# jianhao2016/AllSet

Measured on AMD Instinct MI355X. Metric: edges*d aggregated / sec (V->E->V layer fwd+bwd), higher is better.
Workload: dtype f32

## Files before the change

### allset_amd/csrc/fused_fwd2.hip

```cpp
#include <stdlib.h>

#include "common.h"
#include "mfma.h"

namespace allset {

constexpr int kF2Block = 768;
constexpr int kF2Rows = 32;
constexpr int kF2VWaves = 8;
constexpr int kF2Sets = 4;

#ifdef ALLSET_ABL5_NOBAR
#define ALLSET_TICK() ALLSET_TICK_NO_BARRIER()
#else
#define ALLSET_TICK() ALLSET_TICK_BARRIER()
#endif

template <bool HAS_LN, bool DROP_IN, bool DROP_OUT, bool D8, bool F16, int XM = 0, bool AUX = false>
__global__ __launch_bounds__(kF2Block) void fused_linear_fwd_roles_kernel(
    const float* __restrict__ x, int64_t ldx, const float* __restrict__ gamma, const float* __restrict__ beta, float eps,
    int relu_in, float p_in, uint64_t seed_in, const float* __restrict__ W, const float* __restrict__ bias, int relu_out,
    float p_out, uint64_t seed_out, float* __restrict__ y, int64_t ldy, float* __restrict__ stats, int64_t n,
    const uint64_t* __restrict__ seed_base, uint32_t* __restrict__ mask_out, int64_t xcb, int64_t ycb, float ln_inv,
    const float* __restrict__ colb = nullptr, float* __restrict__ uo = nullptr, int64_t lduo = 0,
// ... 275 lines not shown
        if constexpr (XM == 3 || XM == 4) vv[hb] = v;
#ifdef ALLSET_ABL5_NOSTORE
        if (live && v.x == 123.456f)
#else
        if (live && XM != 2 && XM != 3 && XM != 4)
#endif
          *reinterpret_cast<float4*>(yb + hb * dhy + yo) = v;
        if (mask_out != nullptr) {
          const uint64_t b0 = __ballot(v.x > 0.f), b1 = __ballot(v.y > 0.f), b2 = __ballot(v.z > 0.f), b3 = __ballot(v.w > 0.f);
          const int sh = 8 * (lane0 & 7);
          const uint32_t word = static_cast<uint32_t>((b0 >> sh) & 0xffu) | (static_cast<uint32_t>((b1 >> sh) & 0xffu) << 8) |
                                (static_cast<uint32_t>((b2 >> sh) & 0xffu) << 16) | (static_cast<uint32_t>((b3 >> sh) & 0xffu) << 24);
          if (lane0 < 8 && 16 * (wave >> 2) < nrows)
            mask_out[((stage * (R / 16) + (wave >> 2)) * (ND / 64) + hb) * 32 + (wave & 3) * 8 + lane0] = word;
        }
      }
      if constexpr (XM == 3 || XM == 4) {
        uint32_t u[2][4], own[2] = {0u, 0u}, oth[2] = {0u, 0u};
        int pos[2], kocc;
        const uint32_t sh = 4u * (c & 7);
        const bool hi = c >= 8;
#pragma unroll
        for (int hb = 0; hb < 2; ++hb) {
          u[hb][0] = __float_as_uint(vv[hb].x); u[hb][1] = __float_as_uint(vv[hb].y);
          u[hb][2] = __float_as_uint(vv[hb].z); u[hb][3] = __float_as_uint(vv[hb].w);
        }
        if constexpr (XM == 4) {
          int n2[2];
#pragma unroll
          for (int hb = 0; hb < 2; ++hb)
            n2[hb] = ((u[hb][0] != 0u ? 1 : 0) + (u[hb][1] != 0u ? 1 : 0)) + ((u[hb][2] != 0u ? 1 : 0) + (u[hb][3] != 0u ? 1 : 0));
          const int pk = n2[0] | (n2[1] << 8);
          int inc = pk, tot = pk;
          inc += __builtin_amdgcn_update_dpp(0, inc, 0x111, 0xf, 0xf, true);
          inc += __builtin_amdgcn_update_dpp(0, inc, 0x112, 0xf, 0xf, true);
          inc += __builtin_amdgcn_update_dpp(0, inc, 0x114, 0xf, 0xf, true);
          inc += __builtin_amdgcn_update_dpp(0, inc, 0x118, 0xf, 0xf, true);
          tot += __builtin_amdgcn_update_dpp(0, tot, 0xB1, 0xf, 0xf, false);
          tot += __builtin_amdgcn_update_dpp(0, tot, 0x4E, 0xf, 0xf, false);
          tot += __builtin_amdgcn_update_dpp(0, tot, 0x141, 0xf, 0xf, false);
          tot += __builtin_amdgcn_update_dpp(0, tot, 0x140, 0xf, 0xf, false);
          const int exc = inc - pk, cnt0 = tot & 0xff;
          kocc = cnt0 + (tot >> 8);
          pos[0] = 4 + (exc & 0xff);
          pos[1] = 4 + cnt0 + (exc >> 8);
        } else {
#pragma unroll
          for (int hb = 0; hb < 2; ++hb) {
            const uint32_t nib = (u[hb][0] != 0u ? 1u : 0u) | (u[hb][1] != 0u ? 2u : 0u) | (u[hb][2] != 0u ? 4u : 0u) | (u[hb][3] != 0u ? 8u : 0u);
            float mw = __uint_as_float(nib << sh);
            mw = __uint_as_float(__float_as_uint(mw) | __float_as_uint(dpp_row<0xB1>(mw)));
            mw = __uint_as_float(__float_as_uint(mw) | __float_as_uint(dpp_row<0x4E>(mw)));
            mw = __uint_as_float(__float_as_uint(mw) | __float_as_uint(dpp_row<0x141>(mw)));
            own[hb] = __float_as_uint(mw);
            oth[hb] = __float_as_uint(dpp_row<0x140>(mw));
          }
          const uint32_t below = (1u << sh) - 1u;
          const int cnt0 = __popc(own[0]) + __popc(oth[0]);
          kocc = cnt0 + __popc(own[1]) + __popc(oth[1]);
          pos[0] = 4 + (hi ? __popc(oth[0]) : 0) + __popc(own[0] & below);
          pos[1] = 4 + cnt0 + (hi ? __popc(oth[1]) : 0) + __popc(own[1] & below);
        }
        uint32_t* im = reinterpret_cast<uint32_t*>(sY + (k & 1) * (R * SPY) + lr * SPY);
        __builtin_amdgcn_fence(__ATOMIC_SEQ_CST, "wavefront");
        __builtin_amdgcn_wave_barrier();
        if constexpr (XM == 4) {
          static_assert(kCellCap == 48 && kCellCap + 3 < 64 && 64 + kCellCap + 3 < SPY, "three slots per cell; the staged columns sit 64 dwords above the values");
          const uint32_t dcol = 128u + c;
#pragma unroll
          for (int s = 0; s < 3; ++s) { im[16 * s + c] = 0u; im[64 + 16 * s + c] = dcol; }
#pragma unroll
          for (int hb = 0; hb < 2; ++hb) {
            int j = min(pos[hb] - 4, kCellCap);
#pragma unroll
            for (int i = 0; i < 4; ++i) {
              const bool occ = u[hb][i] != 0u;
              const int at = occ ? j : kCellCap;
              im[at] = u[hb][i];
              im[64 + at] = static_cast<uint32_t>(64 * hb + 4 * c + i);
              j += occ ? 1 : 0;
            }
          }
        } else {
        *reinterpret_cast<uint4*>(im + 4 * c) = make_uint4(0u, 0u, 0u, 0u);
        *reinterpret_cast<uint4*>(im + (hi ? SPY - 4 : 0)) = make_uint4(own[0], oth[0], own[1], oth[1]);
#pragma unroll
        for (int hb = 0; hb < 2; ++hb)
#pragma unroll
          for (int i = 0; i < 4; ++i) {
            const bool occ = u[hb][i] != 0u;
            im[occ ? pos[hb] : SPY - 1] = u[hb][i];
            pos[hb] += occ ? 1 : 0;
          }
        }
        __builtin_amdgcn_fence(__ATOMIC_SEQ_CST, "wavefront");
        __builtin_amdgcn_wave_barrier();
        uint4 o;
        if constexpr (XM == 4)
          o = make_uint4(im[c], im[16 + c], im[32 + c], (im[64 + c] | (im[80 + c] << 8)) | ((im[96 + c] | (static_cast<uint32_t>(kocc) << 8)) << 16));
        else
          o = *reinterpret_cast<const uint4*>(im + 4 * c);
        if (live) *reinterpret_cast<uint4*>(reinterpret_cast<uint32_t*>(uo) + (stage * R + lr) * kPackPitchDw + 4 * c) = o;
        if (live && kocc > (XM == 4 ? kCellCap : kPackCap)) {
          *reinterpret_cast<float4*>(yb + yo) = vv[0];
          *reinterpret_cast<float4*>(yb + 256 + yo) = vv[1];
        }
      }
      if constexpr (XM == 2) {
        __builtin_amdgcn_sched_barrier(0);
        request_res(k + 1);
        __builtin_amdgcn_sched_barrier(0);
      }
    };

    static_assert(kF2Sets == 4, "the trip below is written for four register sets");
#pragma unroll
    for (int q = 0; q < kF2Sets; ++q) request_x(q, xrS[q]);
    request_res(0);
    S0(0, xrS[0]);
    ALLSET_TICK();
    S0(1, xrS[1]);
    ALLSET_TICK();
#define ALLSET_F2_FULL_TICK(tt, set) do { ALLSET_MARK(3); S0((tt) + 1, xrS[set]); ALLSET_MARK(0); E((tt) - 1, eC); ALLSET_MARK(1); ALLSET_TICK(); ALLSET_MARK(2); } while (0)
    int64_t t = 1;
    for (; t + 3 < T; t += 4) {
      ALLSET_F2_FULL_TICK(t, 2);
      ALLSET_F2_FULL_TICK(t + 1, 3);
      ALLSET_F2_FULL_TICK(t + 2, 0);
      ALLSET_F2_FULL_TICK(t + 3, 1);
    }
    if (t < T) ALLSET_F2_FULL_TICK(t, 2);
    if (t + 1 < T) ALLSET_F2_FULL_TICK(t + 1, 3);
    if (t + 2 < T) ALLSET_F2_FULL_TICK(t + 2, 0);
#undef ALLSET_F2_FULL_TICK
    E(T - 1, eB);
  } else {
    const int m = wave - kF2VWaves;
    Frag wq[2][4][F16 ? 2 : 3];
    float inv_s = 1.f;
    if constexpr (F16) {
      const int nn = lane0 & 15, kg = lane0 >> 4;
      float4 wa[2][4], wb[2][4];
      float amax = 0.f;
#pragma unroll
      for (int ct = 0; ct < 2; ++ct)
#pragma unroll
        for (int tt = 0; tt < 4; ++tt) {
          const float4* wr = reinterpret_cast<const float4*>(W + (32 * m + 16 * ct + nn) * KD + 32 * kg + 8 * tt);
          wa[ct][tt] = wr[0]; wb[ct][tt] = wr[1];
          amax = fmaxf(fmaxf(fmaxf(fabsf(wa[ct][tt].x), fabsf(wa[ct][tt].y)), fmaxf(fabsf(wa[ct][tt].z), fabsf(wa[ct][tt].w))), amax);
          amax = fmaxf(fmaxf(fmaxf(fabsf(wb[ct][tt].x), fabsf(wb[ct][tt].y)), fmaxf(fabsf(wb[ct][tt].z), fabsf(wb[ct][tt].w))), amax);
        }
#pragma unroll
      for (int off = 1; off < 64; off <<= 1) amax = fmaxf(amax, __shfl_xor(amax, off));
      const int ew = __builtin_amdgcn_readfirstlane(min(max(static_cast<int>(__float_as_uint(amax) >> 23), 20), 254));
      const float sw = __uint_as_float(static_cast<uint32_t>(254 + 13 - ew) << 23);
      const int X = ew - 140 - Su, X1 = X >> 1, X2 = X - X1;
      inv_s = __uint_as_float(static_cast<uint32_t>(127 + X1) << 23) * __uint_as_float(static_cast<uint32_t>(127 + X2) << 23);
#pragma unroll
      for (int ct = 0; ct < 2; ++ct)
#pragma unroll
        for (int tt = 0; tt < 4; ++tt) {
          const float4 a = wa[ct][tt], b = wb[ct][tt];
          uint32_t ph[4], pl[4];
          split2_f16(a.x * sw, a.y * sw, ph[0], pl[0]);
          split2_f16(a.z * sw, a.w * sw, ph[1], pl[1]);
          split2_f16(b.x * sw, b.y * sw, ph[2], pl[2]);
          split2_f16(b.z * sw, b.w * sw, ph[3], pl[3]);
          wq[ct][tt][0].u = make_uint4(ph[0], ph[1], ph[2], ph[3]);
          wq[ct][tt][1].u = make_uint4(pl[0], pl[1], pl[2], pl[3]);
        }
    } else {
      const int nn = lane0 & 15, kg = lane0 >> 4;
#pragma unroll
      for (int ct = 0; ct < 2; ++ct)
#pragma unroll
// ... 299 lines not shown
```

### allset_amd/csrc/segreduce.hip

```cpp
#include "common.h"
#include "flat_rows.h"
#include "mfma.h"

namespace allset {

enum { kModeSum = 0, kModeExt = 1 };
constexpr int kUnroll = 8;
#ifndef ALLSET_SEG_UNROLL_ONE_SLOT
#define ALLSET_SEG_UNROLL_ONE_SLOT 8
#endif
#ifndef ALLSET_SEG_MAX_LPR
#define ALLSET_SEG_MAX_LPR 64
#endif
constexpr int kBwdUnroll = 4;

template <typename T, int VEC, int LPR, int MODE, bool WEIGHTED>
__global__ __launch_bounds__(kBlock) void segreduce_kernel(
    const int32_t* __restrict__ rowptr, const int32_t* __restrict__ col, const float* __restrict__ w,
    const T* __restrict__ x, int64_t ldx, T* __restrict__ out, int64_t ldo,
    int32_t* __restrict__ argext, int n_t, int d, int mean, float sign, const int32_t* __restrict__ row_order) {
  constexpr int NS = kWave / LPR;
  constexpr int U = NS == 1 ? ALLSET_SEG_UNROLL_ONE_SLOT : kUnroll;
  const unsigned blk = xcd_contiguous_block(blockIdx.x, gridDim.x);
  const int slot_row = static_cast<int>(blk) * kWavesPerBlock + (threadIdx.x >> 6);
// ... 275 lines not shown
        const int jj = j + u * NS + slot;
        const int src = __shfl(my_col, jj & (kWave - 1));
        if (jj < n && active) raw[u] = load_raw<float, VEC>(x + static_cast<int64_t>(src) * ldx + c0);
        else raw[u] = zero_raw<float, VEC>();
      }
      float res = 0.f;
#pragma unroll
      for (int u = 0; u < kUnroll; ++u) {
        const FVec<VEC> v = unpack<float, VEC>(raw[u]);
        float part = 0.f;
#pragma unroll
        for (int k = 0; k < VEC; ++k) {
          if constexpr (MODE == kModeExt) part = (ap[k] == base + j + u * NS + slot) ? fmaf(v.v[k], g.v[k], part) : part;
          else part = fmaf(v.v[k], g.v[k], part);
        }
        part = slot_sum<LPR>(part);
        res = (li == u) ? part : res;
      }
      const int jo = j + li * NS + slot;
      if (li < kUnroll && jo < n) gw[base + jo] = res * scale;
    }
  }
}

constexpr int kPackRowsPerWave = 4;
constexpr int kExpand = 2;

__device__ __forceinline__ void lds_wave_handoff() {
  __builtin_amdgcn_fence(__ATOMIC_SEQ_CST, "wavefront");
  __builtin_amdgcn_wave_barrier();
}

__device__ __forceinline__ uint32_t all_ones_if_bit(uint32_t m, int b) {
  return static_cast<uint32_t>(__builtin_amdgcn_sbfe(static_cast<int>(m), static_cast<unsigned>(b), 1u));
}

__device__ __forceinline__ int mask_count(const uint4& m) { return __popc(m.x) + __popc(m.y) + __popc(m.z) + __popc(m.w); }

template <bool CELLS>
__global__ __launch_bounds__(kBlock) void pack_kernel(const float* __restrict__ x, int64_t ldx, uint32_t* __restrict__ packed, int64_t n) {
  __shared__ __attribute__((aligned(16))) uint32_t image[kWavesPerBlock][kPackRowsPerWave][kPackPitchDw];
  const int wave = threadIdx.x >> 6, lane = lane_id();
  const int slot = lane >> 5, li = lane & 31;
  const int64_t row0 = (static_cast<int64_t>(blockIdx.x) * kWavesPerBlock + wave) * kPackRowsPerWave;
  if (row0 >= n) return;
  uint4 raw[kPackRowsPerWave / 2];
#pragma unroll
  for (int p = 0; p < kPackRowsPerWave / 2; ++p) {
    const int64_t r = row0 + 2 * p + slot;
    raw[p] = r < n ? *reinterpret_cast<const uint4*>(x + r * ldx + 4 * li) : make_uint4(0u, 0u, 0u, 0u);
  }
#pragma unroll
  for (int p = 0; p < kPackRowsPerWave / 2; ++p) {
    uint32_t* dst = image[wave][2 * p + slot];
    const uint32_t v[4] = {raw[p].x, raw[p].y, raw[p].z, raw[p].w};
    const unsigned nib = (v[0] != 0u ? 1u : 0u) | (v[1] != 0u ? 2u : 0u) | (v[2] != 0u ? 4u : 0u) | (v[3] != 0u ? 8u : 0u);
    const int g = li >> 3, sh = 4 * (li & 7);
    unsigned mw = nib << sh;
    mw |= __shfl_xor(mw, 1);
    mw |= __shfl_xor(mw, 2);
    mw |= __shfl_xor(mw, 4);
    uint4 m;
    m.x = __shfl(mw, slot * 32);
    m.y = __shfl(mw, slot * 32 + 8);
    m.z = __shfl(mw, slot * 32 + 16);
    m.w = __shfl(mw, slot * 32 + 24);
    int j = (g > 0 ? __popc(m.x) : 0) + (g > 1 ? __popc(m.y) : 0) + (g > 2 ? __popc(m.z) : 0) + __popc(mw & ((1u << sh) - 1u));
    if constexpr (CELLS) {
      uint8_t* dstb = reinterpret_cast<uint8_t*>(dst);
      const uint32_t k = static_cast<uint32_t>(mask_count(m));
      if (li < kCellsPerRow) *reinterpret_cast<uint4*>(dst + 4 * li) = make_uint4(0u, 0u, 0u, (128u + li) * 0x010101u | (k << 24));
      lds_wave_handoff();
#pragma unroll
      for (int i = 0; i < 4; ++i) {
        if ((nib >> i) & 1u) {
          if (j < kCellCap) {
            dst[4 * (j & 15) + (j >> 4)] = v[i];
            dstb[16 * (j & 15) + 12 + (j >> 4)] = static_cast<uint8_t>(4 * li + i);
          }
          ++j;
        }
      }
    } else {
      int pos = 4 + j;
#pragma unroll
      for (int i = 0; i < 4; ++i) {
        if ((nib >> i) & 1u) {
          if (pos < kPackPitchDw) dst[pos] = v[i];
          ++pos;
        }
      }
      if (li == 0) *reinterpret_cast<uint4*>(dst) = m;
    }
  }
  lds_wave_handoff();
  const int rr = lane >> 4, q = 4 * (lane & 15);
  const uint32_t* src = image[wave][rr];
  uint4 o = *reinterpret_cast<const uint4*>(src + q);
  if constexpr (!CELLS) {
    const int k = mask_count(*reinterpret_cast<const uint4*>(src));
    if (q + 0 >= 4 + k) o.x = 0u;
    if (q + 1 >= 4 + k) o.y = 0u;
    if (q + 2 >= 4 + k) o.z = 0u;
    if (q + 3 >= 4 + k) o.w = 0u;
  }
  if (row0 + rr < n) *reinterpret_cast<uint4*>(packed + (row0 + rr) * kPackPitchDw + q) = o;
}

constexpr int kImagePad = 128;
__global__ __launch_bounds__(kBlock) __attribute__((amdgpu_waves_per_eu(8, 8))) void segreduce_packed_kernel(
    const int32_t* __restrict__ rowptr, const int32_t* __restrict__ col, const uint32_t* __restrict__ packed,
    const float* __restrict__ x, int64_t ldx, float* __restrict__ out, int64_t ldo, int n_t, int mean,
    const int32_t* __restrict__ row_order) {
  constexpr int VEC = 4, LPR = 32, NS = 2, U = kUnroll;
  __shared__ __attribute__((aligned(16))) uint32_t image[kWavesPerBlock * U * NS * kPackPitchDw + kImagePad];
  const unsigned blk = xcd_contiguous_block(blockIdx.x, gridDim.x);
  const int slot_row = static_cast<int>(blk) * kWavesPerBlock + (threadIdx.x >> 6);
  if (slot_row >= n_t) return;
  const int row = row_order ? row_order[slot_row] : slot_row;
  const int wave = threadIdx.x >> 6, lane = lane_id();
  const int slot = lane / LPR, li = lane % LPR;
  const int start = rowptr[row], end = rowptr[row + 1];
  const uint32_t below = (1u << li) - 1u;
  uint32_t* const mine = image + (wave * U * NS + slot) * kPackPitchDw;
  float acc[VEC];
#pragma unroll
  for (int g = 0; g < VEC; ++g) acc[g] = 0.f;

  for (int base = start; base < end; base += kWave) {
    const int n = min(kWave, end - base);
    int my_col = 0;
    if (lane < n) my_col = col[base + lane];
    for (int j = 0; j < n; j += NS * U) {
      uint2 raw[U];
#pragma unroll
      for (int u = 0; u < U; ++u) {
        const int jj = j + u * NS + slot;
        const int src = __shfl(my_col, jj & (kWave - 1));
        if (jj < n) raw[u] = *reinterpret_cast<const uint2*>(packed + static_cast<int64_t>(src) * kPackPitchDw + 2 * li);
        else raw[u] = make_uint2(0u, 0u);
      }
#pragma unroll
      for (int u = 0; u < U; ++u) *reinterpret_cast<uint2*>(mine + u * NS * kPackPitchDw + 2 * li) = raw[u];
      lds_wave_handoff();
#pragma unroll
      for (int u0 = 0; u0 < U; u0 += kExpand) {
        if (j + u0 * NS >= n) break;
        uint4 m[kExpand];
#pragma unroll
        for (int e = 0; e < kExpand; ++e) m[e] = *reinterpret_cast<const uint4*>(mine + (u0 + e) * NS * kPackPitchDw);
        uint32_t v[kExpand][VEC];
        bool over[kExpand];
        bool any_over = false;
#pragma unroll
        for (int e = 0; e < kExpand; ++e) {
          const uint32_t* r = mine + (u0 + e) * NS * kPackPitchDw;
          const int c1 = 4 + __popc(m[e].x), c2 = c1 + __popc(m[e].y), c3 = c2 + __popc(m[e].z);
          over[e] = c3 + __popc(m[e].w) > 4 + kPackCap;
          any_over |= over[e];
          v[e][0] = r[4 + __popc(m[e].x & below)] & all_ones_if_bit(m[e].x, li);
          v[e][1] = r[c1 + __popc(m[e].y & below)] & all_ones_if_bit(m[e].y, li);
          v[e][2] = r[c2 + __popc(m[e].z & below)] & all_ones_if_bit(m[e].z, li);
          v[e][3] = r[c3 + __popc(m[e].w & below)] & all_ones_if_bit(m[e].w, li);
        }
        if (__any(any_over)) {
#pragma unroll
          for (int e = 0; e < kExpand; ++e) {
            const int src = __shfl(my_col, (j + (u0 + e) * NS + slot) & (kWave - 1));
            if (over[e]) {
              const uint32_t* xr = reinterpret_cast<const uint32_t*>(x + static_cast<int64_t>(src) * ldx) + li;
#pragma unroll
              for (int g = 0; g < VEC; ++g) v[e][g] = xr[32 * g];
            }
          }
        }
#pragma unroll
        for (int e = 0; e < kExpand; ++e)
#pragma unroll
          for (int g = 0; g < VEC; ++g) acc[g] = fmaf(1.f, __uint_as_float(v[e][g]), acc[g]);
      }
      lds_wave_handoff();
    }
  }

#pragma unroll
  for (int off = LPR; off < kWave; off <<= 1)
#pragma unroll
    for (int g = 0; g < VEC; ++g) acc[g] += __shfl_xor(acc[g], off);

  if (slot == 0) {
    const float scale = mean ? 1.f / static_cast<float>(max(end - start, 1)) : 1.f;
    float* o = out + static_cast<int64_t>(row) * ldo + li;
#pragma unroll
    for (int g = 0; g < VEC; ++g) o[32 * g] = acc[g] * scale;
  }
}

#ifndef ALLSET_CELL_WAVES
#define ALLSET_CELL_WAVES 8
#endif
constexpr int kCellImageDw = 128 + kCellsPerRow;

__device__ __forceinline__ float add_value_first(uint32_t v, float acc) {
  float r;
  asm("v_add_f32 %0, %1, %2" : "=v"(r) : "v"(v), "v"(acc));
  return r;
}

template <int Q, int H>
__global__ __launch_bounds__(kBlock) __attribute__((amdgpu_waves_per_eu(ALLSET_CELL_WAVES, ALLSET_CELL_WAVES))) void segreduce_cells_kernel(
    const int32_t* __restrict__ rowptr, const int32_t* __restrict__ col, const uint4* __restrict__ cells,
    const float* __restrict__ x, int64_t ldx, float* __restrict__ out, int64_t ldo, int n_t, int mean,
    const int32_t* __restrict__ row_order) {
  static_assert(Q % H == 0, "whole sub-steps");
  constexpr int NI = 4 * H;
  __shared__ __attribute__((aligned(16))) uint32_t image[kWavesPerBlock * NI * kCellImageDw];
  const unsigned blk = xcd_contiguous_block(blockIdx.x, gridDim.x);
  const int slot_row = static_cast<int>(blk) * kWavesPerBlock + (threadIdx.x >> 6);
  if (slot_row >= n_t) return;
  const int row = row_order ? row_order[slot_row] : slot_row;
  const int wave = threadIdx.x >> 6, lane = lane_id();
  const int r4 = lane >> 4, cell = lane & 15;
  const int slot = lane >> 5, li = lane & 31;
  const int start = rowptr[row], end = rowptr[row + 1];
  uint32_t* const wimg = image + wave * NI * kCellImageDw;
  for (int i = lane; i < NI * kCellImageDw / 4; i += kWave) reinterpret_cast<uint4*>(wimg)[i] = make_uint4(0u, 0u, 0u, 0u);
  uint32_t* const wr = wimg + r4 * kCellImageDw;
  const uint32_t* const rd = wimg + slot * kCellImageDw + 4 * li;
  float acc[4] = {0.f, 0.f, 0.f, 0.f};
  lds_wave_handoff();

  for (int base = start; base < end; base += kWave) {
    const int n = min(kWave, end - base);
    int my_col = 0;
    if (lane < n) my_col = col[base + lane];
    for (int j = 0; j < n; j += 4 * Q) {
      uint4 raw[Q];
      uint32_t meta[Q];
      bool ok[Q];
      {
        int src[Q];
#pragma unroll
        for (int q = 0; q < Q; ++q) src[q] = __shfl(my_col, (j + 4 * q + r4) & (kWave - 1));
#pragma unroll
        for (int q = 0; q < Q; ++q) {
          ok[q] = j + 4 * q + r4 < n;
          meta[q] = 0u;
          if (ok[q]) {
            raw[q] = cells[static_cast<int64_t>(src[q]) * kCellsPerRow + cell];
            meta[q] = raw[q].w;
          }
        }
      }
#pragma unroll
      for (int q0 = 0; q0 < Q; q0 += H) {
        if (q0 > 0 && j + 4 * q0 >= n) break;
        bool over[H];
        bool any_over = false;
#pragma unroll
        for (int h = 0; h < H; ++h) {
          uint32_t* im = wr + 4 * h * kCellImageDw;
          const uint32_t m = meta[q0 + h];
          over[h] = (m >> 24) > static_cast<uint32_t>(kCellCap);
          any_over |= over[h];
          if (ok[q0 + h]) {
            im[m & 0xffu] = raw[q0 + h].x;
            im[(m >> 8) & 0xffu] = raw[q0 + h].y;
            im[(m >> 16) & 0xffu] = raw[q0 + h].z;
          }
        }
        any_over = __any(any_over);
// ... 311 lines not shown
```

### include/allset_hip_ext.h

```cpp
#ifndef ALLSET_HIP_EXT_H
#define ALLSET_HIP_EXT_H

#include "allset_hip.h"

#ifdef __cplusplus
extern "C" {
#endif

#define ALLSET_ABI_VERSION 15


int allset_ln_fwd(const float* x, int64_t ldx, const float* gamma, const float* beta, float eps, int relu_in,
                  float p, uint64_t seed, float* y, int64_t ldy, float* stats, int64_t n, int64_t d,
                  const uint64_t* seed_base, void* stream);

int allset_ln_bwd_partials(int64_t n, int64_t d, int64_t* n_partials);
int allset_ln_bwd(const float* gy, int64_t ldg, const float* x, int64_t ldx, const float* stats, const float* gamma,
                  int relu_in, float p, uint64_t seed, float* gx, int64_t ldgx, float* partials, int64_t n_partials,
                  int64_t n, int64_t d, const uint64_t* seed_base, void* stream);

int allset_relu_dropout_fwd(const float* x, float p, uint64_t seed, float* y, int64_t numel,
                            const uint64_t* seed_base, void* stream);
int allset_relu_dropout_bwd(const float* gy, const float* y, float p, float* gx, int64_t numel, void* stream);

// ... 404 lines not shown
                    int64_t n_a, int64_t n_b, int64_t id_base, const int32_t* seeds, int64_t B, int64_t k, uint64_t seed,
                    uint64_t counter, int32_t* endpoints, void* stream);
int allset_han_walk_typed(int metapath, int64_t L, const int32_t* const* rowptrs, const int32_t* const* cols, const int64_t* n_rows,
                          const int32_t* seeds, int64_t B, int64_t k, uint64_t seed, uint64_t counter, int32_t* endpoints,
                          void* stream);
int allset_han_walk_dc(int metapath, const int32_t* rowptr_a, const int32_t* col_a, const int32_t* rowptr_b, const int32_t* col_b,
                       int64_t n_a, int64_t n_b, int64_t id_base, const int32_t* seeds, int64_t B, int64_t k, uint64_t seed,
                       const uint64_t* counter, uint64_t counter_add, int32_t* endpoints, void* stream);
int allset_han_walk_typed_dc(int metapath, int64_t L, const int32_t* const* rowptrs, const int32_t* const* cols, const int64_t* n_rows,
                             const int32_t* seeds, int64_t B, int64_t k, uint64_t seed, const uint64_t* counter, uint64_t counter_add,
                             int32_t* endpoints, void* stream);
int allset_han_block_rows(const int32_t* endpoints, const int32_t* seeds, const int32_t* seeds_sorted, int64_t B, int64_t k,
                          int32_t* rows, int32_t* extra, int32_t* counts, void* stream);
int allset_han_block_fixed_max_slab(int64_t* slots);
int allset_han_block_relabel(const int32_t* counts, const int32_t* extra_sorted, const int32_t* seeds_sorted, int64_t B, int64_t k,
                             int32_t* rowptr, int32_t* uniq, int32_t* sizes, int32_t* status, void* stream);
int allset_han_block_compact_fixed(const int32_t* rows, const int32_t* counts, const int32_t* rowptr, const int32_t* seeds,
                                   const int32_t* seeds_sorted, const int64_t* seed_order, const int32_t* uniq, const int32_t* sizes,
                                   int64_t B, int64_t k, int32_t* col, int32_t* dst, int32_t* key, int64_t* src_ids, void* stream);
int allset_han_block_transpose(const int32_t* keys_sorted, const int64_t* perm, const int32_t* dst, int64_t B, int64_t k,
                               int32_t* rowptrT, int32_t* colT, int32_t* slotT, void* stream);
int allset_han_block_compact(const int32_t* rows, const int32_t* counts, const int32_t* rowptr, const int32_t* seeds_sorted,
                             const int32_t* seed_perm, const int32_t* uniq, int64_t n_extra, int64_t B, int64_t k, int64_t nnz,
                             int32_t* col, int32_t* dst, void* stream);
int allset_han_block_hop_fwd(int64_t nnz, const int32_t* rowptr, const int32_t* col, const float* el, const float* er, const float* x,
                             int64_t ldx, float slope, const float* bias, float p_att, uint64_t seed, const uint64_t* seed_base,
                             float* y, int64_t ldy, float* outpos, int64_t ldpos, float* ppos, float* lse, int64_t n_dst,
                             int64_t n_src, int64_t H, int64_t C, void* stream);
int allset_han_block_hop_bwd_stats(const float* y, int64_t ldy, const float* bias, const float* gy, int64_t ldgy, const float* outpos,
                                   int64_t ldpos, const float* ppos, const float* lse, float slope, float* g, int64_t ldg,
                                   float* stats, float* ger, int64_t n_dst, int64_t H, int64_t C, void* stream);
int allset_han_block_hop_bwd_src(int64_t nnz, const int32_t* rowptrT, const int32_t* colT, const int32_t* slotT, const float* el,
                                 const float* er, const float* x, int64_t ldx, const float* g, int64_t ldg, const float* stats,
                                 float slope, float p_att, uint64_t seed, const uint64_t* seed_base, float* gx, int64_t ldgx,
                                 float* gel, int64_t n_dst, int64_t n_src, int64_t H, int64_t C, void* stream);

int allset_hattn_supported(void);
int allset_hattn_coef(int64_t nnz, const int32_t* rowptr, const int32_t* col, const int32_t* perm, const int32_t* pos, const float* av,
                      const float* ae, float slope, float p, uint64_t seed, const uint64_t* seed_base, float* a_v, float* a_e,
                      float* m, float* l, int64_t n_v, int64_t n_e, int64_t H, void* stream);
int allset_hattn_hop(int64_t nnz, const int32_t* row_order, const int32_t* rowptr, const int32_t* col, const float* w, const float* r,
                     const float* s, const float* x, int64_t ldx, const float* bias, int act, float p, uint64_t seed,
                     const uint64_t* seed_base, int concat, float* y, int64_t ldy, int64_t n_t, int64_t n_s, int64_t H, int64_t C,
                     void* stream);
int allset_hattn_bwd_vertex(int64_t nnz, const int32_t* rowptr, const int32_t* col, const int32_t* pos, const float* a_v,
                            const float* av, const float* ae, const float* m, const float* l, float slope, const float* z, int64_t ldz,
                            const float* g_u, int64_t ldg, const float* y, int64_t ldy, const float* gy, int64_t ldgy, const float* D,
                            const float* B, float* gz, int64_t ldgz, float* t, float* gav, float* ge_e, int64_t n_v, int64_t n_e,
                            int64_t H, int64_t C, void* stream);
int allset_hattn_bwd_edge(int64_t nnz, const int32_t* rowptr, const float* ge_e, float* gae, int64_t n_e, int64_t H, void* stream);

int allset_spgemm_bool_bins(int64_t* bins );
int allset_spgemm_bool_workspace_bytes(int64_t n_a, size_t* bytes);
int allset_spgemm_bool_count(const int32_t* rowptrA, const int32_t* colA, const int32_t* rowptrB, const int32_t* colB, int64_t n_a,
                             int64_t n_b, int64_t n_c, int32_t* cnt, void* workspace, size_t workspace_bytes, void* stream);
int allset_spgemm_bool_fill(const int32_t* rowptrA, const int32_t* colA, const int32_t* rowptrB, const int32_t* colB, int64_t n_a,
                            int64_t n_b, int64_t n_c, const int32_t* rowptrC, int64_t nnz_c, int32_t* colC, const void* workspace,
                            size_t workspace_bytes, void* stream);

int allset_loo_supported(int64_t d);
int allset_loo_long_threshold(void);
int allset_loo_rows(const int32_t* rowptr, const int32_t* col, const float* src, int64_t lds, const float* s_src, const float* s_seg,
                    float* out, int64_t ldo, const int32_t* long_seg, int64_t n_long, int64_t n_seg, int64_t n_src, int64_t nnz,
                    int64_t d, void* stream);

int allset_loo_softmax_supported(int64_t d, int64_t heads);
int allset_loo_softmax_fwd(const int32_t* rowptr, const int32_t* col, const float* alpha, const float* V, int64_t ldv, float slope,
                           float* out, int64_t ldo, float* lse, const int32_t* long_seg, int64_t n_long, int64_t n_seg,
                           int64_t n_src, int64_t nnz, int64_t d, int64_t heads, void* stream);
int allset_loo_softmax_bwd(const int32_t* rowptr, const int32_t* col, const float* alpha, const float* V, int64_t ldv, float slope,
                           const float* out, int64_t ldo, const float* lse, const float* gout, int64_t ldg, const float* glse,
                           float* gV, int64_t ldgv, float* galpha, float* scratch, const int32_t* long_seg, int64_t n_long,
                           int64_t n_seg, int64_t n_src, int64_t nnz, int64_t d, int64_t heads, void* stream);

int allset_scan_rows_supported(int64_t d);
int allset_scan_rows(const int32_t* rowptr, const int32_t* col, const float* src, int64_t lds, const float* s_src, float* out,
                     int64_t ldo, const int32_t* long_seg, int64_t n_long, int reverse, int64_t n_seg, int64_t n_src, int64_t nnz,
                     int64_t d, void* stream);
int allset_scan_collect(const int32_t* rowptr, const int32_t* col, const float* t, int64_t ldt, const float* r_self, const float* x,
                        int64_t ldx, const float* s, const float* bias, int act, float p, uint64_t seed, const uint64_t* seed_base,
                        float* y, int64_t ldy, int64_t n_t, int64_t n_pos, int64_t d, int64_t width, void* stream);

enum { kPackPitchDw = 64, kPackCap = 60 };
int allset_pack_rows_f32(const float* x, int64_t ldx, void* packed, int64_t n, int64_t d, void* stream);
int allset_segreduce_packed_fwd(int reduce, const int32_t* row_order, const int32_t* rowptr, const int32_t* col, const void* packed,
                                const float* x, int64_t ldx, float* out, int64_t ldo, int64_t n_t, int64_t n_s, int64_t d, void* stream);

int allset_fused_linear_fwd_packed_supported(int64_t K, int64_t N, int has_ln, float p_in, float p_out);
int allset_fused_linear_fwd_packed(const float* x, int64_t ldx, const float* gamma, const float* beta, float eps, int relu_in,
                                   float p_in, uint64_t seed_in, const float* W, const float* bias, int relu_out, float p_out,
                                   uint64_t seed_out, void* packed, float* side, int64_t ldside, float* stats, int64_t n, int64_t K,
                                   int64_t N, const uint64_t* seed_base, uint32_t* mask_out, int arith, void* stream);

enum { kCellsPerRow = 16, kCellCap = 48 };
int allset_pack_cells_f32(const float* x, int64_t ldx, void* cells, int64_t n, int64_t d, void* stream);
int allset_segreduce_cells_fwd(int reduce, const int32_t* row_order, const int32_t* rowptr, const int32_t* col, const void* cells,
                               const float* x, int64_t ldx, float* out, int64_t ldo, int64_t n_t, int64_t n_s, int64_t d, void* stream);
int allset_fused_linear_fwd_cells_supported(int64_t K, int64_t N, int has_ln, float p_in, float p_out);
int allset_fused_linear_fwd_cells(const float* x, int64_t ldx, const float* gamma, const float* beta, float eps, int relu_in, float p_in,
                                  uint64_t seed_in, const float* W, const float* bias, int relu_out, float p_out, uint64_t seed_out,
                                  void* cells, float* side, int64_t ldside, float* stats, int64_t n, int64_t K, int64_t N,
                                  const uint64_t* seed_base, uint32_t* mask_out, int arith, void* stream);

#ifdef __cplusplus
}
#endif
#endif
```

Baseline: 255.8 billion.

## Annotate packed sparse rows with scatter slots and add a fast-path expansion

When a row has at most 47 nonzeros, the packed row format now also carries a byte table of destination slots plus a signature word. Both the producer kernels (the fused linear forward and pack_rows) write this annotation. The packed segment-reduce kernel checks the signature and takes a fast path: it loads whole 16-byte cells, scatters the values into zeroed LDS images using the precomputed slots, then accumulates and clears the images. This replaces the per-lane mask-rank expansion, but adds extra LDS barriers and zeroing passes and uses a different LDS layout. Accumulation also switches to an inline-asm v_add_f32 in place of fmaf(1, v, acc).

```diff
diff --git a/allset_amd/csrc/fused_fwd2.hip b/allset_amd/csrc/fused_fwd2.hip
--- a/allset_amd/csrc/fused_fwd2.hip
+++ b/allset_amd/csrc/fused_fwd2.hip
@@ -381,16 +381,28 @@
             }
           }
         } else {
+        static_assert(kPackAnnByte == 204 && kPackAnnSigDw == 63 && (kPackAnnByte + 56 + 128) / 4 < SPY - 4, "the annotation's stores");
+        const bool ann = kocc <= kPackAnnCap;
+        const uint32_t dW = 0x83828180u;
         *reinterpret_cast<uint4*>(im + 4 * c) = make_uint4(0u, 0u, 0u, 0u);
+        *reinterpret_cast<uint4*>(im + 4 * c + (ann && c >= 13 ? 0 : 64)) = make_uint4(dW + 0x04040404u, dW + 0x08080808u, dW + 0x0C0C0C0Cu, dW);
+        im[ann && c < 2 ? (c == 0 ? kPackAnnByte / 4 : kPackAnnSigDw) : 64 + c] = c == 0 ? dW : ALLSET_PACK_ANN_SIG(static_cast<uint32_t>(kocc));
         *reinterpret_cast<uint4*>(im + (hi ? SPY - 4 : 0)) = make_uint4(own[0], oth[0], own[1], oth[1]);
-#pragma unroll
-        for (int hb = 0; hb < 2; ++hb)
+        uint8_t* const imb = reinterpret_cast<uint8_t*>(im) + kPackAnnByte;
+        const uint32_t slot0 = 16u * (c & 7) + (c >> 3);
+        const int junk = 52 + 4 * c;
+#pragma unroll
+        for (int hb = 0; hb < 2; ++hb) {
+          int rank = pos[hb] - 4 + (ann ? 0 : 56);
 #pragma unroll
           for (int i = 0; i < 4; ++i) {
             const bool occ = u[hb][i] != 0u;
             im[occ ? pos[hb] : SPY - 1] = u[hb][i];
+            imb[occ ? rank : junk] = static_cast<uint8_t>(slot0 + 2 * hb + 4 * i);
             pos[hb] += occ ? 1 : 0;
+            rank += occ ? 1 : 0;
           }
+        }
         }
         __builtin_amdgcn_fence(__ATOMIC_SEQ_CST, "wavefront");
         __builtin_amdgcn_wave_barrier();
diff --git a/allset_amd/csrc/segreduce.hip b/allset_amd/csrc/segreduce.hip
--- a/allset_amd/csrc/segreduce.hip
+++ b/allset_amd/csrc/segreduce.hip
@@ -381,11 +381,19 @@
         }
       }
     } else {
+      uint8_t* dstb = reinterpret_cast<uint8_t*>(dst);
+      const uint32_t k = static_cast<uint32_t>(mask_count(m));
+      const bool ann = k <= static_cast<uint32_t>(kPackAnnCap);
+      if (ann && li < 12) dst[kPackAnnByte / 4 + li] = 0x83828180u + static_cast<uint32_t>((4 * li) & 15) * 0x01010101u;
+      if (ann && li == 12) dst[kPackAnnSigDw] = ALLSET_PACK_ANN_SIG(k);
+      lds_wave_handoff();
+      const uint32_t slot0 = 16u * (li & 7) + (li >> 3);
       int pos = 4 + j;
 #pragma unroll
       for (int i = 0; i < 4; ++i) {
         if ((nib >> i) & 1u) {
           if (pos < kPackPitchDw) dst[pos] = v[i];
+          if (ann) dstb[kPackAnnByte - 4 + pos] = static_cast<uint8_t>(slot0 + 4u * i);
           ++pos;
         }
       }
@@ -398,49 +406,130 @@
   uint4 o = *reinterpret_cast<const uint4*>(src + q);
   if constexpr (!CELLS) {
     const int k = mask_count(*reinterpret_cast<const uint4*>(src));
-    if (q + 0 >= 4 + k) o.x = 0u;
-    if (q + 1 >= 4 + k) o.y = 0u;
-    if (q + 2 >= 4 + k) o.z = 0u;
-    if (q + 3 >= 4 + k) o.w = 0u;
+    const int tail = k <= kPackAnnCap ? kPackAnnByte / 4 : kPackPitchDw;
+    if (q + 0 >= 4 + k && q + 0 < tail) o.x = 0u;
+    if (q + 1 >= 4 + k && q + 1 < tail) o.y = 0u;
+    if (q + 2 >= 4 + k && q + 2 < tail) o.z = 0u;
+    if (q + 3 >= 4 + k && q + 3 < tail) o.w = 0u;
   }
   if (row0 + rr < n) *reinterpret_cast<uint4*>(packed + (row0 + rr) * kPackPitchDw + q) = o;
 }
 
-constexpr int kImagePad = 128;
+__device__ __forceinline__ float add_sum_first(float acc, uint32_t v) {
+  float r;
+  asm("v_add_f32 %0, %1, %2" : "=v"(r) : "v"(acc), "v"(v));
+  return r;
+}
+
+constexpr int kAnnImageDw = 128 + 16;
 __global__ __launch_bounds__(kBlock) __attribute__((amdgpu_waves_per_eu(8, 8))) void segreduce_packed_kernel(
     const int32_t* __restrict__ rowptr, const int32_t* __restrict__ col, const uint32_t* __restrict__ packed,
     const float* __restrict__ x, int64_t ldx, float* __restrict__ out, int64_t ldo, int n_t, int mean,
     const int32_t* __restrict__ row_order) {
   constexpr int VEC = 4, LPR = 32, NS = 2, U = kUnroll;
-  __shared__ __attribute__((aligned(16))) uint32_t image[kWavesPerBlock * U * NS * kPackPitchDw + kImagePad];
+  constexpr int Q = 4, H = 2, NI = 4 * H;
+  constexpr int kWaveDw = NI * kAnnImageDw;
+  static_assert(NS * U == 4 * Q, "a step is 16 incidences either way");
+  static_assert((NS * U - 1) * kPackPitchDw + 4 + 128 <= kWaveDw, "the raw rows and their stray reads fit the wave's images");
+  __shared__ __attribute__((aligned(16))) uint32_t image[kWavesPerBlock * kWaveDw];
   const unsigned blk = xcd_contiguous_block(blockIdx.x, gridDim.x);
-  const int slot_row = static_cast<int>(blk) * kWavesPerBlock + (threadIdx.x >> 6);
+  const int wave = __builtin_amdgcn_readfirstlane(static_cast<int>(threadIdx.x >> 6)), lane = lane_id();
+  const int slot_row = static_cast<int>(blk) * kWavesPerBlock + wave;
   if (slot_row >= n_t) return;
   const int row = row_order ? row_order[slot_row] : slot_row;
-  const int wave = threadIdx.x >> 6, lane = lane_id();
   const int slot = lane / LPR, li = lane % LPR;
+  const int r4 = lane >> 4, cell = lane & 15;
+  const bool value_lane = cell >= 1 && cell <= 12;
   const int start = rowptr[row], end = rowptr[row + 1];
   const uint32_t below = (1u << li) - 1u;
-  uint32_t* const mine = image + (wave * U * NS + slot) * kPackPitchDw;
+  uint32_t* const wimg = image + wave * kWaveDw;
+  uint32_t* const mine = wimg + slot * kPackPitchDw;
+  uint32_t* const wr = wimg + r4 * kAnnImageDw;
+  const uint32_t* const rd = wimg + slot * kAnnImageDw + 4 * li;
   float acc[VEC];
 #pragma unroll
   for (int g = 0; g < VEC; ++g) acc[g] = 0.f;
+  for (int i = lane; i < kWaveDw / 4; i += kWave) reinterpret_cast<uint4*>(wimg)[i] = make_uint4(0u, 0u, 0u, 0u);
+  lds_wave_handoff();
 
   for (int base = start; base < end; base += kWave) {
     const int n = min(kWave, end - base);
     int my_col = 0;
     if (lane < n) my_col = col[base + lane];
     for (int j = 0; j < n; j += NS * U) {
-      uint2 raw[U];
-#pragma unroll
-      for (int u = 0; u < U; ++u) {
-        const int jj = j + u * NS + slot;
-        const int src = __shfl(my_col, jj & (kWave - 1));
-        if (jj < n) raw[u] = *reinterpret_cast<const uint2*>(packed + static_cast<int64_t>(src) * kPackPitchDw + 2 * li);
-        else raw[u] = make_uint2(0u, 0u);
-      }
-#pragma unroll
-      for (int u = 0; u < U; ++u) *reinterpret_cast<uint2*>(mine + u * NS * kPackPitchDw + 2 * li) = raw[u];
+      uint4 raw[Q];
+      bool ok[Q];
+      bool bad = false;
+      {
+        int src[Q];
+#pragma unroll
+        for (int q = 0; q < Q; ++q) src[q] = __shfl(my_col, (j + 4 * q + r4) & (kWave - 1));
+#pragma unroll
+        for (int q = 0; q < Q; ++q) {
+          ok[q] = j + 4 * q + r4 < n;
+          if (ok[q]) raw[q] = *reinterpret_cast<const uint4*>(packed + static_cast<int64_t>(src[q]) * kPackPitchDw + 4 * cell);
+        }
+#pragma unroll
+        for (int q = 0; q < Q; ++q) {
+          const uint32_t sig = static_cast<uint32_t>(__builtin_amdgcn_update_dpp(0, static_cast<int>(raw[q].w), 0x121, 0xf, 0xf, false));
+          const uint32_t k = static_cast<uint32_t>(mask_count(raw[q]));
+          const uint32_t diff = (sig ^ ALLSET_PACK_ANN_SIG(0u)) ^ (k | (k << 8));
+          bad |= ok[q] && (diff != 0u || k > static_cast<uint32_t>(kPackAnnCap));
+        }
+      }
+      if (!__any(cell == 0 && bad)) {
+#pragma unroll
+        for (int q0 = 0; q0 < Q; q0 += H) {
+          if (q0 > 0 && j + 4 * q0 >= n) break;
+#pragma unroll
+          for (int h = 0; h < H; ++h)
+            if (cell >= 12) *reinterpret_cast<uint4*>(wr + 4 * h * kAnnImageDw + 128 + 4 * (cell - 12)) = raw[q0 + h];
+          lds_wave_handoff();
+          uint32_t sl[H];
+#pragma unroll
+          for (int h = 0; h < H; ++h)
+            sl[h] = wr[4 * h * kAnnImageDw + 128 + ((kPackAnnByte / 4 - 48 - 1 + cell) & 15)];
+#pragma unroll
+          for (int h = 0; h < H; ++h) {
+            uint32_t* im = wr + 4 * h * kAnnImageDw;
+            if (value_lane && ok[q0 + h]) {
+              im[sl[h] & 0xffu] = raw[q0 + h].x;
+              im[(sl[h] >> 8) & 0xffu] = raw[q0 + h].y;
+              im[(sl[h] >> 16) & 0xffu] = raw[q0 + h].z;
+              im[sl[h] >> 24] = raw[q0 + h].w;
+            }
+          }
+          lds_wave_handoff();
+#pragma unroll
+          for (int u0 = 0; u0 < 2 * H; u0 += 2) {
+            uint4 v[2];
+#pragma unroll
+            for (int e = 0; e < 2; ++e) v[e] = *reinterpret_cast<const uint4*>(rd + 2 * (u0 + e) * kAnnImageDw);
+#pragma unroll
+            for (int e = 0; e < 2; ++e) {
+              acc[0] = add_sum_first(acc[0], v[e].x);
+              acc[1] = add_sum_first(acc[1], v[e].y);
+              acc[2] = add_sum_first(acc[2], v[e].z);
+              acc[3] = add_sum_first(acc[3], v[e].w);
+            }
+          }
+          lds_wave_handoff();
+#pragma unroll
+          for (int h = 0; h < H; ++h)
+            if (value_lane && ok[q0 + h]) {
+              uint32_t* im = wr + 4 * h * kAnnImageDw;
+              im[sl[h] & 0xffu] = 0u;
+              im[(sl[h] >> 8) & 0xffu] = 0u;
+              im[(sl[h] >> 16) & 0xffu] = 0u;
+              im[sl[h] >> 24] = 0u;
+            }
+          lds_wave_handoff();
+        }
+        continue;
+      }
+#pragma unroll
+      for (int q = 0; q < Q; ++q)
+        *reinterpret_cast<uint4*>(wimg + (4 * q + r4) * kPackPitchDw + 4 * cell) = ok[q] ? raw[q] : make_uint4(0u, 0u, 0u, 0u);
       lds_wave_handoff();
 #pragma unroll
       for (int u0 = 0; u0 < U; u0 += kExpand) {
@@ -476,8 +565,10 @@
 #pragma unroll
         for (int e = 0; e < kExpand; ++e)
 #pragma unroll
-          for (int g = 0; g < VEC; ++g) acc[g] = fmaf(1.f, __uint_as_float(v[e][g]), acc[g]);
-      }
+          for (int g = 0; g < VEC; ++g) acc[g] = add_sum_first(acc[g], v[e][g]);
+      }
+      lds_wave_handoff();
+      for (int i = lane; i < kWaveDw / 4; i += kWave) reinterpret_cast<uint4*>(wimg)[i] = make_uint4(0u, 0u, 0u, 0u);
       lds_wave_handoff();
     }
   }
@@ -485,7 +576,7 @@
 #pragma unroll
   for (int off = LPR; off < kWave; off <<= 1)
 #pragma unroll
-    for (int g = 0; g < VEC; ++g) acc[g] += __shfl_xor(acc[g], off);
+    for (int g = 0; g < VEC; ++g) acc[g] = add_sum_first(acc[g], __float_as_uint(__shfl_xor(acc[g], off)));
 
   if (slot == 0) {
     const float scale = mean ? 1.f / static_cast<float>(max(end - start, 1)) : 1.f;
diff --git a/include/allset_hip_ext.h b/include/allset_hip_ext.h
--- a/include/allset_hip_ext.h
+++ b/include/allset_hip_ext.h
@@ -510,6 +510,9 @@
                         float* y, int64_t ldy, int64_t n_t, int64_t n_pos, int64_t d, int64_t width, void* stream);
 
 enum { kPackPitchDw = 64, kPackCap = 60 };
+enum { kPackAnnCap = 47, kPackAnnByte = 204, kPackAnnSigDw = 63 };
+#define ALLSET_PACK_ANN_SIG(k) (0xA55A0000u | ((unsigned)(k) << 8) | (~(unsigned)(k) & 0xffu))
+#define ALLSET_PACK_ANN_SLOT(c) (4u * ((unsigned)(c) & 31u) + ((unsigned)(c) >> 5))
 int allset_pack_rows_f32(const float* x, int64_t ldx, void* packed, int64_t n, int64_t d, void* stream);
 int allset_segreduce_packed_fwd(int reduce, const int32_t* row_order, const int32_t* rowptr, const int32_t* col, const void* packed,
                                 const float* x, int64_t ldx, float* out, int64_t ldo, int64_t n_t, int64_t n_s, int64_t d, void* stream);
```

Measured after the change: 257.2 billion (median of 6 runs). No clear change (+0.6%).
